# lmb-freiburg/locov

Hardware: AMD Instinct MI355X
Metric: proposals/sec through LSM ROI-head (1333x800, 1000 prop, 1203-class text bank) (higher is better)
Workload: dtype f32 (Res5 GEMM products formed from f16x2 split operands on the f16 matrix pipe, f32 accumulate; error vs f64 <= 1.5 x the f32-MFMA kernel's + 6e-7 and <= 3e-6 on every tested shape, tests/test_gpu_split_gemm.py)

## Files before the change

include/locov_hip.h:

```cpp
#ifndef LOCOV_HIP_H
#define LOCOV_HIP_H

#include <stdint.h>

#ifdef __cplusplus
extern "C" {
#endif

#define LOCOV_ABI_VERSION 8

#define LOCOV_OK 0
#define LOCOV_ERR_INVALID_ARG (-1)
#define LOCOV_ERR_LAUNCH (-2)
#define LOCOV_ERR_UNSUPPORTED (-3)

#define LOCOV_F32 0
#define LOCOV_BF16 1

#define LOCOV_NORM_NONE 0
#define LOCOV_NORM_L2 1
#define LOCOV_NORM_STANDARDIZE 2

#define LOCOV_EPI_RELU 1u
#define LOCOV_GEMM_A_SPLIT 0x1000u
// ... 428 lines not shown
} locov_weight_prep_job;
int locov_res5_weight_prep(const locov_weight_prep_job *jobs, int n_jobs, unsigned *overflow, locov_stream_t stream);

int locov_weight_transpose_scale(const float *w, int N, int K, const float *row_scale, float *out,
                                 locov_stream_t stream);
int locov_conv3x3_weight_flip(const float *w, int N, int Cin, const float *row_scale, float *out,
                              locov_stream_t stream);
int locov_im2col3x3_nhwc(const float *x, int64_t R, int H, int W, int C, float *col, locov_stream_t stream);
int locov_conv3x3_wgrad_unpack(const float *dw_packed, int N, int Cin, const float *row_scale, float *dw,
                               locov_stream_t stream);
int locov_relu_mask(const float *g, const float *act, int64_t n, float *out, float *amax_out, locov_stream_t stream);
#define LOCOV_ZERO_LIST_MAX 24
int locov_zero_if_raised(float *const *tensors, const int64_t *counts, int n_tensors, const unsigned *flag,
                         locov_stream_t stream);

int locov_spatial_mean_bwd(const float *g, const float *act, int64_t R, int C, int HW, float *out,
                           float *amax_out, locov_stream_t stream);
int locov_rows_stride2(const float *src, int N, int H, int W, int C, int forward, float *dst,
                       locov_stream_t stream);
int locov_roi_align_nhwc_bwd(const float *grad_rows, int64_t grad_ld, int N, int H, int W, int C,
                             const float *rois, int64_t R, int pooled_h, int pooled_w, float spatial_scale,
                             int sampling_ratio, int aligned, int bin_stride, int pos_major, float *grad_feat,
                             locov_stream_t stream);

#define LOCOV_REGIONS_MAX_B 64
#define LOCOV_REGIONS_MAX_CANDIDATES 4096
#define LOCOV_REGIONS_GRID 0
#define LOCOV_REGIONS_GRID_ALL 1
#define LOCOV_REGIONS_BOXES 2
#define LOCOV_REGIONS_ROWS 0
#define LOCOV_REGIONS_NCHW 1
int locov_regions_select(const double *keys, int mode, int B, const int *count_host, const int *ext_a_host,
                         const int *ext_b_host, int grid_w, const float *const *boxes_host, int n, int limit, int mask_w,
                         int mvm_w, int64_t *indices, int *src_row, int *inv, uint8_t *mask, float *loc, float *mvm,
                         locov_stream_t stream);
int locov_regions_gather_fwd(const float *src, int layout, int64_t ld, int B, int n, int C, int64_t hw, const int *src_row,
                             float *out, locov_stream_t stream);
int locov_regions_gather_bwd(const float *grad_out, int layout, int64_t ld, int64_t rows, int C, int64_t hw, const int *inv,
                             float *grad_src, locov_stream_t stream);

#define LOCOV_MHA_MAX_S 4096
#define LOCOV_MHA_MAX_GRID 65535
int locov_mha_fwd(const float *q, int64_t ldq, const float *k, int64_t ldk, const float *v, int64_t ldv, const float *bias,
                  const uint8_t *keep, float p_drop, float scale, int nseq, int S, int H, int d, float *ctx, int64_t ldo,
                  float *lse, locov_stream_t stream);
int locov_mha_bwd(const float *q, int64_t ldq, const float *k, int64_t ldk, const float *v, int64_t ldv, const float *bias,
                  const uint8_t *keep, float p_drop, float scale, int nseq, int S, int H, int d, const float *dctx,
                  int64_t ldo, const float *lse, float *delta, float *dq, int64_t lddq, float *dk, int64_t lddk, float *dv,
                  int64_t lddv, locov_stream_t stream);

int locov_resnet_stem_fwd(const float *x, int N, int H, int W, const float *w, const float *scale, const float *shift, int Cout,
                          float *y, locov_stream_t stream);

#ifdef __cplusplus
}
#endif
#endif
```

locov_amd/_lib.py:

```python
from __future__ import annotations

import ctypes
import os
from ctypes import c_char_p, c_double, c_float,c_int, c_int64, c_uint, c_void_p, POINTER

HERE = os.path.dirname(os.path.abspath(__file__))
LIB_PATH = os.environ.get("LOCOV_HIP_LIB") or os.path.join(HERE, "liblocov_hip.so")

OK = 0
F32, BF16 = 0, 1
NORM_NONE, NORM_L2, NORM_STANDARDIZE = 0, 1, 2
EPI_RELU = 1
WINO_OUT_ROI_MAJOR = 0x100
WINO_IN_ROI_MAJOR = 0x200
SEGMEAN_RES_ROI_MAJOR = 0x400
GEMM_A_SPLIT = 0x1000
EPI_OUT_SPLIT = 0x2000
EPI_RES_SPLIT = 0x4000
MAX_LEVELS = 8
ZERO_LIST_MAX = 24
LABEL_MAX_IMAGES, LABEL_MAX_THRESHOLDS, SAMPLE_MAX_PROPOSALS = 64, 6, 4096
ABI_VERSION = 8
DETECT_MAX_CANDIDATES, DETECT_FLAG_NONFINITE, DETECT_FLAG_OVERFLOW = 8192, 1, 2
RPN_FLAG_NONFINITE, RPN_MAX_PRE_NMS_TOPK, RPN_MAX_ANCHORS = 1, 16384, (1 << 22) - 1
RPN_LOSS_FLAG_DEGENERATE = 1
FED_LOSS_MAX_CLASSES = 32767
DISTILL_KD, DISTILL_JS, DISTILL_MSE, DISTILL_MAX_B = 0, 1, 2, 64
GROUNDING_ALIGN_SOFTMAX, GROUNDING_ALIGN_HARDMAX = 0, 1
TRIPLET_HARDEST, TRIPLET_EASIEST, TRIPLET_GIVEN = 0, 1, 2
BOX_IOU_GIOU, BOX_IOU_DIOU, BOX_IOU_CIOU = 0, 1, 2
REGIONS_MAX_B, REGIONS_MAX_CANDIDATES = 64, 4096
REGIONS_GRID, REGIONS_GRID_ALL, REGIONS_BOXES = 0, 1, 2
REGIONS_ROWS, REGIONS_NCHW = 0, 1
MHA_MAX_S, MHA_MAX_GRID, MHA_HEAD_DIMS = 4096, 65535, (32, 64, 96, 128)

_p = c_void_p

WEIGHT_PREP_MAX_JOBS = 32
AMAX_BOUND_MAX = 4
PREP_PLAIN, PREP_TRANSPOSE, PREP_IM2COL, PREP_IM2COL_FLIP, PREP_WINO, PREP_WINO_FLIP = range(6)


class WeightPrepJob(ctypes.Structure):
    _fields_ = [("w", c_void_p), ("row_scale", c_void_p), ("out", c_void_p), ("scale", c_float), ("kind", c_int), ("N", c_int), ("K", c_int)]


SIGNATURES = {
    "locov_abi_version": (c_int, []),
    "locov_last_error": (c_char_p, []),
    "locov_launch_count": (c_int64, []),
    "locov_device_info": (c_int, [POINTER(c_int), POINTER(c_int), POINTER(c_int)]),
    "locov_level_assign": (c_int, [_p, c_int64, c_int, c_int, c_int, c_int, _p, _p]),
    "locov_roi_align_fwd": (c_int, [_p, c_int, c_int, c_int, c_int, _p, c_int64, c_int, c_int, c_float,
                                    c_int, c_int, _p, _p]),
    "locov_roi_align_bwd": (c_int, [_p, c_int, c_int, c_int, c_int, _p, c_int64, c_int, c_int, c_float,
                                    c_int, c_int, _p, _p]),
    "locov_roi_align_levels_fwd": (c_int, [POINTER(c_void_p), POINTER(c_int), POINTER(c_int), POINTER(c_float),
                                           c_int, c_int, c_int, _p, _p, c_int64, c_int, c_int, c_int, c_int,
                                           _p, _p]),
    "locov_nchw_to_nhwc": (c_int, [_p, c_int, c_int, c_int, c_int, _p, c_int, _p]),
    "locov_roi_align_nhwc_fwd": (c_int, [_p, c_int, c_int, c_int, c_int, c_int, _p, c_int64, c_int, c_int,
                                         c_float, c_int, c_int, c_int, c_int, _p, c_int, _p]),
    "locov_roi_align_nhwc_ld_fwd": (c_int, [_p, c_int, c_int, c_int, c_int, c_int, _p, c_int64, c_int, c_int,
                                            c_float, c_int, c_int, c_int, c_int, _p, c_int64, c_int, _p]),
    "locov_roi_align_nhwc_affine_fwd": (c_int, [_p, c_int, c_int, c_int, c_int, c_int, c_int64, _p, c_int64, c_int, c_int,
                                                c_float, c_int, c_int, c_int, c_int, _p, _p, c_int, _p, c_int64, c_int, _p]),
    "locov_roi_align_from_nhwc_fwd": (c_int, [_p, c_int, c_int, c_int, c_int, _p, c_int64, c_int, c_int, c_float,
                                              c_int, c_int, _p, _p]),
    "locov_roi_align_plan_bytes": (c_int64, [c_int64]),
    "locov_roi_align_from_nhwc_fwd_ex": (c_int, [_p, c_int, c_int, c_int, c_int, _p, c_int64, c_int, c_int, c_float,
                                                 c_int, c_int, c_int, _p, c_int64, _p, _p]),
    "locov_spatial_mean_fwd": (c_int, [_p, c_int64, c_int, c_int, c_int, _p, _p]),
    "locov_gemm_nt_f32": (c_int, [_p, c_int64, _p, _p, _p, _p, _p, c_int64, c_int64, c_int, c_int, c_uint, _p]),
    "locov_conv3x3_nhwc_f32": (c_int, [_p, c_int64, c_int, c_int, c_int, c_int, _p, _p, _p, _p, _p, c_int, c_uint,
                                       _p]),
    "locov_pack_conv3x3_weight": (c_int, [_p, c_int, c_int, _p, c_int, _p]),
    "locov_winograd_workspace_bytes": (c_int64, [c_int64, c_int, c_int]),
    "locov_winograd_pack_weight": (c_int, [_p, c_int, c_int, _p, _p]),
    "locov_winograd_conv3x3_f32": (c_int, [_p, c_int64, c_int, _p, _p, _p, _p, c_int64, c_int, c_uint, _p, c_int64, _p]),
    "locov_winograd_conv3x3_f32_split": (c_int, [_p, c_int64, c_int, _p, c_float, c_float, _p, _p, _p, c_int64, c_int, c_uint,
                                                 _p, c_int64, _p, _p]),
    "locov_gemm_nt_batched_f32": (c_int, [_p, c_int64, c_int64, _p, c_int64, _p, c_int64, c_int64, c_int64, c_int,
                                          c_int, c_int, _p]),
    "locov_gemm_timing_enable": (c_int, [c_int]),
    "locov_gemm_timing_read": (c_int, [c_int, _p, _p, _p]),
    "locov_gemm_timing_read_ex": (c_int, [c_int, _p, _p, _p, _p]),
    "locov_frozen_bn_fold": (c_int, [_p, _p, _p, _p, c_float, c_int, _p, _p, _p]),
    "locov_label_proposals": (c_int, [_p, POINTER(c_int), _p, _p, POINTER(c_int), c_int, POINTER(c_float), POINTER(c_float),
                                      POINTER(c_int), c_int, c_int64, _p, _p, _p, _p, _p, _p, _p]),
    "locov_sample_proposals": (c_int, [_p, _p, _p, _p, _p, _p, _p, _p, POINTER(c_int), POINTER(c_int), c_int, c_int, c_int, c_int64,
                                       _p, _p, _p, _p, _p, _p, _p, _p]),
    "locov_box_reg_loss": (c_int, [_p, _p, _p, c_int64, _p, c_int64, c_int64, c_float, c_float, c_float, c_float, c_float, _p, _p, _p]),
    "locov_box_iou_loss": (c_int, [_p, _p, _p, c_int64, _p, c_int64, c_int64, c_float, c_float, c_float, c_float, c_double, c_int, _p, _p,
                                   _p]),
    "locov_cls_loss_workspace_bytes": (c_int64, [c_int64]),
    "locov_cls_loss": (c_int, [_p, c_int64, _p, c_int64, c_int, c_int64, _p, c_int64, _p, _p, _p, _p]),
    "locov_fed_loss_classes": (c_int, [_p, c_int64, _p, _p, c_int, c_int, _p, _p, _p]),
# ... 59 lines not shown
                                                c_int, c_int, c_float, c_float, _p, _p]),
    "locov_sim_gemm_bf16": (c_int, [_p, _p, c_int64, c_int, c_int, _p, c_int64, _p]),
    "locov_gemm_nt_f32_ex": (c_int, [_p, c_int64, _p, c_int64, _p, _p, _p, _p, _p, c_int64, c_int64, c_int, c_int, c_uint, _p]),
    "locov_conv3x3_nhwc_f32_ex": (c_int, [_p, c_int64, c_int, c_int, c_int, c_int, _p, _p, _p, _p, _p, _p, c_int, c_uint, _p]),
    "locov_winograd_conv3x3_f32_ex": (c_int, [_p, c_int64, c_int, _p, _p, _p, _p, _p, c_int64, c_int, c_uint, _p, c_int64, _p]),
    "locov_gemm_tn_workspace_bytes": (c_int64, [c_int64, c_int, c_int, c_int]),
    "locov_gemm_tn_f32": (c_int, [_p, c_int64, c_int64, _p, c_int64, c_int64, _p, c_int64, c_int64, c_int64, c_int, c_int, c_int,
                                  _p, _p, c_int64, _p]),
    "locov_split_scale_from_amax": (c_int, [_p, c_int64, c_float, _p, _p]),
    "locov_amax_bound": (c_int, [POINTER(c_void_p), POINTER(c_int64), POINTER(c_float), c_int, _p, _p]),
    "locov_split_scale_from_amax_zeroed": (c_int, [_p, c_int64, c_float, _p, _p]),
    "locov_gemm_nt_f32_split_ex": (c_int, [_p, c_int64, _p, _p, _p, _p, _p, _p, c_int64, c_int64, c_int, c_int, c_uint, c_float, _p,
                                           c_float, _p, _p, _p]),
    "locov_gemm_tn_f32_split": (c_int, [_p, c_int64, c_int64, _p, c_int64, c_int64, _p, c_int64, c_int64, c_int64, c_int, c_int, c_int,
                                        _p, _p, c_float, _p, _p, c_int64, _p]),
    "locov_gemm_tn_f32_split_b": (c_int, [_p, c_int64, c_int64, _p, c_int64, c_int64, _p, c_int64, c_int64, c_int64, c_int, c_int, c_int,
                                        _p, _p, c_float, _p, _p, c_int64, _p]),
    "locov_winograd_conv3x3_f32_split_ex": (c_int, [_p, c_int64, c_int, _p, c_float, c_float, c_int, _p, _p, _p, _p, c_int64, c_int,
                                                    c_uint, c_float, _p, c_int64, _p, _p, _p]),
    "locov_winograd_wgrad_f32_split": (c_int, [_p, _p, c_int64, c_int, c_int, c_uint, _p, _p, _p, _p, c_int64, _p]),
    "locov_winograd_wgrad_f32_split_v": (c_int, [_p, _p, c_int64, c_int, c_int, c_uint, _p, _p, _p, _p, c_int64, _p]),
    "locov_conv1x1_winograd_workspace_bytes": (c_int64, [c_int64, c_int, c_int]),
    "locov_conv1x1_winograd_workspace_bytes_for": (c_int64, [c_int64, c_int, c_int, c_int, c_int64]),
    "locov_roi_align_winograd_workspace_bytes": (c_int64, [c_int64, c_int, c_int]),
    "locov_roi_align_winograd_conv3x3_f32_split": (c_int, [_p, c_int, c_int, c_int, c_int, c_int64, _p, c_int64, c_int, c_float, c_int, c_int,
                                                           _p, _p, _p, c_float, c_float, _p, _p, _p, c_int64, c_int, c_uint, c_float, _p, c_int64,
                                                           _p, _p]),
    "locov_conv1x1_winograd_conv3x3_f32_split": (c_int, [_p, c_int64, c_int, c_float, _p, c_float, _p, _p, c_int64, c_int, _p, c_float, c_float,
                                                         _p, _p, _p, c_int64, c_int, c_uint, c_float, _p, c_int64, _p, _p]),
    "locov_winograd_wgrad_workspace_bytes": (c_int64, [c_int64, c_int, c_int]),
    "locov_winograd_wgrad_f32": (c_int, [_p, _p, c_int64, c_int, c_int, c_uint, _p, _p, _p, c_int64, _p]),
    "locov_res5_weight_prep": (c_int, [POINTER(WeightPrepJob), c_int, _p, _p]),
    "locov_weight_transpose_scale": (c_int, [_p, c_int, c_int, _p, _p, _p]),
    "locov_conv3x3_weight_flip": (c_int, [_p, c_int, c_int, _p, _p, _p]),
    "locov_im2col3x3_nhwc": (c_int, [_p, c_int64, c_int, c_int, c_int, _p, _p]),
    "locov_conv3x3_wgrad_unpack": (c_int, [_p, c_int, c_int, _p, _p, _p]),
    "locov_relu_mask": (c_int, [_p, _p, c_int64, _p, _p, _p]),
    "locov_zero_if_raised": (c_int, [POINTER(c_void_p), POINTER(c_int64), c_int, _p, _p]),
    "locov_spatial_mean_bwd": (c_int, [_p, _p, c_int64, c_int, c_int, _p, _p, _p]),
    "locov_rows_stride2": (c_int, [_p, c_int, c_int, c_int, c_int, c_int, _p, _p]),
    "locov_roi_align_nhwc_bwd": (c_int, [_p, c_int64, c_int, c_int, c_int, c_int, _p, c_int64, c_int, c_int, c_float, c_int, c_int,
                                         c_int, c_int, _p, _p]),
    "locov_box_head_fwd": (c_int, [_p, c_int64, c_int, c_int, c_int, _p, _p, _p, _p, _p, _p, c_int, c_int,
                                   c_int, c_int, _p, _p, _p, _p, _p, _p]),
    "locov_regions_select": (c_int, [_p, c_int, c_int, POINTER(c_int), POINTER(c_int), POINTER(c_int), c_int, POINTER(c_void_p), c_int, c_int,
                                     c_int, c_int, _p, _p, _p, _p, _p, _p, _p]),
    "locov_regions_gather_fwd": (c_int, [_p, c_int, c_int64, c_int, c_int, c_int, c_int64, _p, _p, _p]),
    "locov_regions_gather_bwd": (c_int, [_p, c_int, c_int64, c_int64, c_int, c_int64, _p, _p, _p]),
    "locov_mha_fwd": (c_int, [_p, c_int64, _p, c_int64, _p, c_int64, _p, _p, c_float, c_float, c_int, c_int, c_int, c_int, _p, c_int64,
                              _p, _p]),
    "locov_mha_bwd": (c_int, [_p, c_int64, _p, c_int64, _p, c_int64, _p, _p, c_float, c_float, c_int, c_int, c_int, c_int, _p,
                              c_int64, _p, _p, _p, c_int64, _p, c_int64, _p, c_int64, _p]),
    "locov_resnet_stem_fwd": (c_int, [_p, c_int, c_int, c_int, _p, _p, _p, c_int, _p, _p]),
}

_lib = None


class LocovError(RuntimeError):
    pass


def load() -> ctypes.CDLL:
    global _lib
    if _lib is not None:
        return _lib
    if not os.path.exists(LIB_PATH):
        raise LocovError(
            f"{LIB_PATH} not found: build it with `python -m locov_amd.build` "
            "(or __graft_entry__.build()).  The LSM ROI-head path has no fallback.")
    lib = ctypes.CDLL(LIB_PATH)
    for name, (restype, argtypes) in SIGNATURES.items():
        try:
            fn = getattr(lib, name)
        except AttributeError as e:
            raise LocovError(f"{LIB_PATH} does not export {name}") from e
        fn.restype = restype
        fn.argtypes = argtypes
    if lib.locov_abi_version() != ABI_VERSION:
        raise LocovError(f"ABI version mismatch: library {lib.locov_abi_version()} != binding {ABI_VERSION}")
    _lib = lib
    return lib


def check(rc: int, what: str = "") -> None:
    if rc != OK:
        msg = load().locov_last_error()
        raise LocovError(f"{what or 'liblocov_hip'} failed (code {rc}): {msg.decode() if msg else ''}")
```

locov_amd/res5.py:

```python
from __future__ import annotations

from typing import Optional

import torch
import torch.nn.functional as F
from torch import nn

import os

from .res5_operands import Res5Operands, TrainOperands

_OUT_SPLIT = os.environ.get("LOCOV_RES5_OUT_SPLIT", "1") != "0"
_FUSE12 = os.environ.get("LOCOV_RES5_FUSE12", "1") != "0"


class FrozenBatchNorm2d(nn.Module):

    def __init__(self, num_features: int, eps: float = 1e-5):
        super().__init__()
        self.num_features = num_features
        self.eps = eps
        self.register_buffer("weight", torch.ones(num_features))
        self.register_buffer("bias", torch.zeros(num_features))
        self.register_buffer("running_mean", torch.zeros(num_features))
        self.register_buffer("running_var", torch.ones(num_features) - eps)

    def scale_shift(self):
        scale = self.weight * (self.running_var + self.eps).rsqrt()
        shift = self.bias - self.running_mean * scale
        return scale, shift

    def forward(self, x):
        scale, shift = self.scale_shift()
        return x * scale.reshape(1, -1, 1, 1) + shift.reshape(1, -1, 1, 1)


class Conv2d(nn.Conv2d):

    def __init__(self, *args, norm: Optional[nn.Module] = None, **kwargs):
        super().__init__(*args, **kwargs)
        self.norm = norm

    def forward(self, x):
        x = F.conv2d(x, self.weight, self.bias, self.stride, self.padding, self.dilation, self.groups)
        if self.norm is not None:
            x = self.norm(x)
        return x


def get_norm(norm: str, ch: int):
    if norm in ("FrozenBN", "FrozenBatchNorm2d"):
        return FrozenBatchNorm2d(ch)
    if norm in ("", None):
        return None
    if norm == "BN":
        return nn.BatchNorm2d(ch)
    raise ValueError(f"unsupported norm {norm!r} for the Res5 head")


class BottleneckBlock(nn.Module):
    def __init__(self, in_channels, out_channels, *, bottleneck_channels, stride=1, num_groups=1,
                 norm="FrozenBN", stride_in_1x1=True):
        super().__init__()
        self.in_channels, self.out_channels, self.stride = in_channels, out_channels, stride
        self.stride_in_1x1 = stride_in_1x1
        if in_channels != out_channels:
            self.shortcut = Conv2d(in_channels, out_channels, kernel_size=1, stride=stride, bias=False,
                                   norm=get_norm(norm, out_channels))
        else:
            self.shortcut = None
        s1, s3 = (stride, 1) if stride_in_1x1 else (1, stride)
        self.conv1 = Conv2d(in_channels, bottleneck_channels, kernel_size=1, stride=s1, bias=False,
                            norm=get_norm(norm, bottleneck_channels))
        self.conv2 = Conv2d(bottleneck_channels, bottleneck_channels, kernel_size=3, stride=s3, padding=1,
                            bias=False, groups=num_groups, norm=get_norm(norm, bottleneck_channels))
        self.conv3 = Conv2d(bottleneck_channels, out_channels, kernel_size=1, bias=False,
                            norm=get_norm(norm, out_channels))
        for layer in (self.conv1, self.conv2, self.conv3, self.shortcut):
            if layer is not None:
                nn.init.kaiming_normal_(layer.weight, mode="fan_out", nonlinearity="relu")

    def forward(self, x):
        out = F.relu_(self.conv1(x))
        out = F.relu_(self.conv2(out))
        out = self.conv3(out)
        shortcut = self.shortcut(x) if self.shortcut is not None else x
        out = out + shortcut
        return F.relu_(out)


class Res5Stage(nn.Sequential):

    def __init__(self, *blocks):
        super().__init__(*blocks)
        self.operands = Res5Operands(self)
        self._guards = {}
        self._warned = set()

    def range_guard(self, kind: str, device):
        from . import ops
        key = (kind, torch.device(device), torch.cuda.current_stream(device).cuda_stream)
        g = self._guards.get(key)
        if g is None:
            g = self._guards[key] = ops.RangeGuard(device, deferred=kind in self.DEFERRED_KINDS)
        return g

    DEFERRED_KINDS = ("bwd", "fwd_train")

    def deferred_guards(self, device):
        dev = torch.device(device)
        return [(kind, g) for (kind, d, _), g in self._guards.items() if kind in self.DEFERRED_KINDS and d == dev]

    def backward_guard_words(self, device):
        return [g.word for kind, g in self.deferred_guards(device) if kind == "bwd"]

    def forget_scales(self) -> None:
        self.operands.forget_scales()

    def backward_guard_tripped(self) -> None:
        self.forget_scales()
        for (kind, _, _), g in self._guards.items():
            if kind == "bwd":
                g.reset()

    def backward_guard_raised(self, device) -> bool:
        words = self.backward_guard_words(device)
        hit = bool(words) and bool(int(torch.stack([w.reshape(()) for w in words]).max()))
        if hit:
            self.backward_guard_tripped()
        return hit

    def supports_rows_path(self) -> bool:
        b0 = self[0]
        return (all(isinstance(c.norm, FrozenBatchNorm2d) for blk in self for c in
                    (blk.conv1, blk.conv2, blk.conv3)) and b0.stride_in_1x1 and all(blk.conv2.groups == 1 for blk in self))

    def train_operands(self, split: bool, grid: bool = True, rois: bool = True) -> TrainOperands:
        return self.operands.train_operands(split, grid, rois)

    def rows_input(self, M: int, device) -> torch.Tensor:
        b0 = self[0]
        cin, mid = b0.conv1.in_channels, b0.conv1.out_channels
        if b0.shortcut is None or not self.supports_rows_path() or mid % 4 or cin % 4:
            return torch.empty((M, cin), dtype=torch.float32, device=device)
        buf = torch.empty((M, mid + cin), dtype=torch.float32, device=device)
        x0 = buf[:, mid:]
        x0._locov_cat = buf
        return x0

    def _linear(self, split: bool, x, conv, bias=None, tag: str = "plain", **kw):
        from . import ops
        w = self.operands.for_gemm(conv, tag, split)
        if isinstance(w, ops.SplitWeight):
            return ops.linear_split(x, w, bias, **kw)
        assert not (kw.get("x_is_split") or kw.get("out_split") or kw.get("residual_is_split")), \
            "a split-layout activation needs the split GEMM"
        for k in ("x_is_split", "x_scale", "out_split", "residual_is_split"):
            kw.pop(k, None)
        return ops.linear(x, w, bias, **kw)

    def _warn_once(self, key: str, text: str) -> None:
        if key not in self._warned:
            self._warned.add(key)
            import warnings
            warnings.warn(text, RuntimeWarning, stacklevel=3)

    ACT_SPLIT_SCALE = 16.0

    def _y2_split_ok(self, split: bool, c2, w3) -> bool:
        return bool(split) and c2.out_channels % 32 == 0 and w3.shape[1] % 32 == 0 and w3.shape[0] % 4 == 0

    def _out_split_ok(self, split: bool, winograd: bool, bi: int, pooled: bool) -> bool:
        if not (split and winograd) or bi + 1 >= len(self) or not _OUT_SPLIT:
            return False
        nxt, cur = self[bi + 1], self[bi]
        ch = cur.conv3.out_channels
        return (nxt.shortcut is None and ch % 32 == 0 and nxt.conv1.out_channels % 4 == 0 and nxt.conv3.out_channels % 8 == 0
                and nxt.conv2.in_channels % 32 == 0 and nxt.conv2.out_channels % 4 == 0)

    def map_path_pays(self, n_rois: int, n_pixels: int) -> bool:
        b0 = self[0]
        return (b0.shortcut is not None and self.supports_rows_path() and b0.conv1.in_channels % 32 == 0
                and b0.conv1.out_channels % 32 == 0 and 49 * n_rois >= 3 * n_pixels)

    @torch.no_grad()
    def forward_from_map(self, nhwc: torch.Tensor, rois: torch.Tensor, pooler_resolution: int, spatial_scale: float,
                         sampling_ratio: int = 0, aligned: bool = True, winograd: bool = True,
                         bf16: bool = False, split: bool = False, pooled: bool = False, roi_major: bool = False) -> torch.Tensor:
        from . import ops
        assert self.supports_rows_path() and self[0].shortcut is not None and pooler_resolution == 14
        b0 = self[0]
        mid = b0.conv1.out_channels
        N, H, W, cin = nhwc.shape
        P = self.operands
        wmap, shift_tail, (s1, b1) = P.get(b0, "on_map"), P.get(b0, "on_map", "shift"), P.fold(b0.conv1)
        if bf16:
            g = ops.linear_bf16(ops.to_bf16(nhwc.reshape(N * H * W, cin)), P.get(b0, "on_map", "bf16")).view(N, H, W, wmap.shape[0])
        else:
            g = self._linear(split, nhwc.reshape(N * H * W, cin), b0, tag="on_map").view(N, H, W, wmap.shape[0])
        pm = not (roi_major and not bf16)
        c2 = b0.conv2
        w3, s3, (s2, b2) = P.get(b0.conv3, "plain"), P.fold(b0.conv3)[0], P.fold(c2)
        use_wino = winograd and c2.in_channels % 32 == 0 and c2.out_channels % 4 == 0
        fuse_pool = _FUSE12 and split and use_wino and not bf16 and not pm and g.dtype == torch.float32
        R = rois.shape[0]
        y = None
        if not fuse_pool:
            y = ops.roi_align_nhwc(g[..., :mid], rois, 14, spatial_scale, sampling_ratio, aligned, bin_stride=2,
                                   pos_major=pm, ch_scale=s1, ch_shift=b1, relu=True).view(49 * R, mid)
        sc = ops.roi_align_nhwc(g[..., mid:], rois, 14, spatial_scale, sampling_ratio, aligned, bin_stride=2,
                                pos_major=pm).view(49 * R, -1)
        if bf16:
            y = ops.conv3x3_nhwc_bf16(ops.to_bf16(y), P.get(c2, "col", "bf16"), 7, 7, scale=s2, shift=b2, relu=True, pos_major=True)
            x = ops.linear_bf16(ops.to_bf16(y), P.get(b0.conv3, "plain", "bf16"), shift_tail, scale=s3, residual=sc, relu=True)
            return self.forward_rows(x, 7, 7, pos_major=True, start_block=1, bf16=True)
        y_split = False
        if use_wino:
            u2 = P.get(c2, "wino", "split" if split else "fp32")
            y_split = self._y2_split_ok(split, c2, w3)
            if fuse_pool:
                y = ops.roi_align_winograd_conv3x3(g[..., :mid], rois, 14, spatial_scale, sampling_ratio, aligned, u2,
                                                   ch_scale=s1, ch_shift=b1, scale2=s2, shift2=b2, relu=True, roi_major=True,
                                                   out_split_scale=self.ACT_SPLIT_SCALE if y_split else None)
            else:
                y = ops.winograd_conv3x3(y, u2, scale=s2, shift=b2, relu=True, roi_major=not pm, in_roi_major=not pm,
                                         out_split_scale=self.ACT_SPLIT_SCALE if y_split else None)
        else:
            y = ops.conv3x3_nhwc(y, P.get(c2, "col"), 7, 7, scale=s2, shift=b2, relu=True, pos_major=pm)
        x_split = self._out_split_ok(split, winograd, 0, pooled)
        kw3 = {"x_is_split": True, "x_scale": self.ACT_SPLIT_SCALE} if y_split else {}
        if x_split:
            kw3.update(out_split=True, x_scale=self.ACT_SPLIT_SCALE)
        x = self._linear(split, y, b0.conv3, shift_tail, scale=s3, residual=sc, relu=True, **kw3)
        return self.forward_rows(x, 7, 7, pos_major=pm, winograd=winograd, start_block=1, split=split, pooled=pooled,
                                 x0_is_split=x_split)

    @torch.no_grad()
    def forward_rows(self, x0: torch.Tensor, H: int, W: int, pos_major: bool = False,
                     winograd: bool = True, start_block: int = 0, bf16: bool = False, split: bool = False,
                     pooled: bool = False, x0_is_split: bool = False) -> torch.Tensor:
        from . import ops
        assert self.supports_rows_path(), "forward_rows needs FrozenBN, STRIDE_IN_1X1 and ungrouped convs"
        x = x0
        x_split = bool(x0_is_split)
        assert not x_split or (split and start_block > 0)
        cat = getattr(x0, "_locov_cat", None)
        P = self.operands
        for bi, blk in enumerate(self):
            if bi < start_block:
                continue
            c2 = blk.conv2
            w1, w3 = P.get(blk.conv1, "plain"), P.get(blk.conv3, "plain")
            (s1, b1), (s2, b2), (s3, b3) = P.fold(blk.conv1), P.fold(c2), P.fold(blk.conv3)
            if bf16:
                y = ops.linear_bf16(ops.to_bf16(x.contiguous()), P.get(blk.conv1, "plain", "bf16"), b1, scale=s1, relu=True)
                y = ops.conv3x3_nhwc_bf16(ops.to_bf16(y), P.get(c2, "col", "bf16"), H, W, scale=s2, shift=b2, relu=True,
                                          pos_major=pos_major)
                if blk.shortcut is not None:
                    ss, bs = P.fold(blk.shortcut)
                    sc = ops.linear_bf16(ops.to_bf16(x.contiguous()), P.get(blk.shortcut, "plain", "bf16"), bs, scale=ss)
                else:
                    sc = x
                x = ops.linear_bf16(ops.to_bf16(y), P.get(blk.conv3, "plain", "bf16"), b3, scale=s3, residual=sc, relu=True)
                continue
            xs_kw = {"x_is_split": True, "x_scale": self.ACT_SPLIT_SCALE} if x_split else {}
            use_wino = winograd and H == 7 and W == 7 and c2.in_channels % 32 == 0 and c2.out_channels % 4 == 0
            assert use_wino or not x_split
            rm = not pos_major
            fuse12 = _FUSE12 and x_split and use_wino and rm and w1.shape[0] % 32 == 0

            def conv12(**kw):
                u2 = P.get(c2, "wino", "split" if split else "fp32")
                if fuse12:
                    return ops.conv1x1_winograd_conv3x3(x, P.get(blk.conv1, "plain", "split"), b1, u2, scale1=s1, scale2=s2, shift2=b2,
                                                        relu=True, x_scale=self.ACT_SPLIT_SCALE, roi_major=kw["roi_major"],
                                                        out_split_scale=kw.get("out_split_scale"))
                return ops.winograd_conv3x3(y, u2, scale=s2, shift=b2, relu=True, in_roi_major=rm, **kw)

            y = None if fuse12 else self._linear(split, x, blk.conv1, b1, scale=s1, relu=True, **xs_kw)
            if use_wino and bi == 0 and cat is not None and blk.shortcut is not None:
                ops.winograd_conv3x3(y, P.get(c2, "wino", "split" if split else "fp32"), scale=s2, shift=b2, relu=True,
                                     out=cat[:, :c2.out_channels], roi_major=rm, in_roi_major=rm)
                x = self._linear(split, cat, blk, P.get(blk, "tail", "shift"), tag="tail", relu=True)
                continue
            last = bi == len(self) - 1
            if use_wino and pooled and last and split and blk.shortcut is None and w3.shape[1] % 32 == 0 and w3.shape[0] % 4 == 0:
                ysp = self._y2_split_ok(True, c2, w3)
                if not ops.segmean_supported(x.shape[0], w3.shape[0], w3.shape[1], H * W, residual_roi_major=rm, x_is_split=ysp,
                                             residual_is_split=x_split):
# ... 52 lines not shown
```

locov_amd/roi_heads/roi_emb_heads.py:

```python
from __future__ import annotations

import os
from typing import Dict, List, Optional

import torch
from torch import nn

from .. import ops
from ..poolers import ROIPooler, convert_boxes_to_pooler_format
from ..registry import Registry, configurable
from ..res5 import build_res5_block
from ..structures import Boxes, ShapeSpec
from .box_emb_head import build_box_predictor
from .labelling import (_EVENTS, Matcher, ROIHeads, SampleAllROIHeads, add_ground_truth_to_proposals, get_event_storage,
                        subsample_labels, subsample_order)

ROI_HEADS_REGISTRY = Registry("ROI_HEADS")
_JOINT_FORWARD = os.environ.get("LOCOV_RES5_JOINT_FWD", "1") != "0"

__all__ = ["ROI_HEADS_REGISTRY", "build_roi_heads", "Matcher", "subsample_labels", "add_ground_truth_to_proposals",
           "ROIHeads", "SampleAllROIHeads", "EmbeddingRes5ROIHeads", "EmbeddingProposalsRes5ROIHeads"]


@ROI_HEADS_REGISTRY.register()
# ... 189 lines not shown
                and self._train_path_ok(feats) and self._needs_graph(feats) and hasattr(self.res5, "range_guard")):
            return None
        if ops.active_guard(feats[0].device) is not None:
            return None
        g = self.res5.range_guard("fwd_train", feats[0].device)
        g.step_word = torch.zeros(1, dtype=torch.int32, device=feats[0].device)
        return g

    @staticmethod
    def _close_train_guard(tguard, outputs, losses=None):
        tguard.step_word.copy_(tguard.word)
        ops.zero_if_raised(list(outputs), tguard.step_word)
        return (tguard.step_word == 0).to(torch.float32).reshape(())

    def _backward_guard_tripped(self) -> None:
        import warnings
        self.res5.backward_guard_tripped()
        warnings.warn("a remembered split-operand weight scale stopped covering its weight during the previous step's Res5 backward "
                      "(weights grew 8x within 64 steps): that backward's Res5 gradients were ZEROED on the device (the step was "
                      "skipped for the Res5 weights and the feature map, GradScaler-style; no inf / NaN was applied); the scales "
                      "are chosen afresh from here on", RuntimeWarning, stacklevel=3)

    def _warn_overflow(self):
        if hasattr(self.res5, "forget_scales"):
            self.res5.forget_scales()
        if not self._overflow_warned:
            import warnings
            warnings.warn("Res5 activations left the range of the f16x2 split arithmetic (|x| >= 4094): this call was repeated "
                          "on the f32 MFMA (RES5_DTYPE 'fp32' avoids the retry; reported once per module)", RuntimeWarning, stacklevel=3)
            self._overflow_warned = True

    def _fused_roi_transform(self, features, boxes, pooled, res5_dtype):
        assert len(boxes) == features[0].shape[0]
        rois = convert_boxes_to_pooler_format(boxes)
        P = self.pooler.output_size[0]
        nhwc = ops.nchw_to_nhwc(features[0].detach())
        oh = ow = P // 2
        R = rois.shape[0]
        wino = self.res5_conv3x3 == "winograd"
        split = res5_dtype == "f16x2"
        if res5_dtype == "bf16":
            x0 = torch.empty((oh * ow * R, nhwc.shape[3]), dtype=torch.float32, device=nhwc.device)
            if P == 14 and self.res5[0].shortcut is not None:
                y = self.res5.forward_from_map(nhwc, rois, P, self.pooler.scales[0], self.pooler.sampling_ratio,
                                               self.pooler.aligned, bf16=True)
            else:
                ops.roi_align_nhwc(nhwc, rois, P, self.pooler.scales[0], self.pooler.sampling_ratio, self.pooler.aligned,
                                   bin_stride=2, pos_major=True, out=x0)
                y = self.res5.forward_rows(x0, oh, ow, pos_major=True, bf16=True)
            y = y.view(oh, ow, R, y.shape[1]).permute(2, 3, 0, 1)
            return self._pooled_mean(y) if pooled else y
        if P == 14 and self.res5.map_path_pays(R, nhwc.shape[0] * nhwc.shape[1] * nhwc.shape[2]):
            y = self.res5.forward_from_map(nhwc, rois, P, self.pooler.scales[0], self.pooler.sampling_ratio,
                                           self.pooler.aligned, winograd=wino, split=split, pooled=pooled, roi_major=wino)
            if pooled:
                return y
            return y.view(R, oh, ow, y.shape[1]).permute(0, 3, 1, 2) if wino else y.view(oh, ow, R, y.shape[1]).permute(2, 3, 0, 1)
        x0 = self.res5.rows_input(oh * ow * R, nhwc.device)
        pm = not (wino and oh == 7)
        ops.roi_align_nhwc(nhwc, rois, P, self.pooler.scales[0], self.pooler.sampling_ratio, self.pooler.aligned,
                           bin_stride=2, pos_major=pm, out=x0)
        y = self.res5.forward_rows(x0, oh, ow, pos_major=pm, winograd=wino, split=split, pooled=pooled)
        if pooled:
            return y
        return y.view(oh, ow, R, y.shape[1]).permute(2, 3, 0, 1) if pm else y.view(R, oh, ow, y.shape[1]).permute(0, 3, 1, 2)

    def _pooled_mean(self, box_features: torch.Tensor) -> torch.Tensor:
        if torch.is_grad_enabled() and box_features.requires_grad:
            return box_features.mean(dim=[2, 3])
        if not box_features.is_contiguous():
            if box_features.permute(2, 3, 0, 1).is_contiguous():
                return ops.spatial_mean(box_features.permute(2, 3, 0, 1), channels_last=2)
            if box_features.permute(0, 2, 3, 1).is_contiguous():
                return ops.spatial_mean(box_features.permute(0, 2, 3, 1), channels_last=1)
        return ops.spatial_mean(box_features)

    def forward(self, images, features, proposals, targets=None):
        del images
        if not self.training:
            del targets
            return self._detect(features, proposals)
        assert targets
        pending = self._label_begin(proposals, targets)
        del targets
        feats = [features[f] for f in self.in_features]
        del features

        def attempt(sampled):
            props = sampled if sampled is not None else self._label_finish(pending)
            proposal_boxes = [x.proposal_boxes for x in props]
            tguard = self._train_guard(feats)
            guard = None if tguard is not None else self._deferred_guard(feats)
            with ops.range_guard(tguard if tguard is not None else guard):
                box_features = self._shared_roi_transform(feats, proposal_boxes, pooled=True,
                                                          rois=pending["rois"] if pending.get("rois_of") is props else None)
            keep = None
            if tguard is not None:
                keep = self._close_train_guard(tguard, [box_features])
            elif guard is not None and guard.event is None:
                guard.snapshot()
            predictions = self.box_predictor(box_features)
            losses = self._predictor_losses(predictions, props)
            if keep is not None:
                losses = {k: v * keep for k, v in losses.items()}
            return props, losses, guard

        dtype_was = self.res5_dtype
# ... 164 lines not shown
```

Before: 393,900.

## Run the Res5 forward-from-map chain in one native call, optionally split across two streams

Adds a native res5 chain entry point that runs the on-map GEMM, ROI-align-Winograd, and the three bottleneck blocks' fused kernels from a single cached argument table. The goal is to remove Python and ctypes dispatch overhead for each stage. It can also cut the ROIs into two halves and pipeline them on a side stream offset by one stage, so kernels from the two halves overlap. INFER_SEGMENTS defaults to 1, so the default path does no split and the gain comes mainly from lower host overhead. The two-stream path adds a mutex, events, and more workspace.

```diff
diff --git a/include/locov_hip.h b/include/locov_hip.h
--- a/include/locov_hip.h
+++ b/include/locov_hip.h
@@ -504,6 +504,30 @@
 int locov_resnet_stem_fwd(const float *x, int N, int H, int W, const float *w, const float *scale, const float *shift, int Cout,
                           float *y, locov_stream_t stream);
 
+typedef struct locov_res5_chain_block {
+    const void *w1, *u2, *w3;
+    float w1_scale, u2_scale, w3_scale, pad_;
+    const float *s1, *b1, *s2, *b2, *s3, *b3;
+} locov_res5_chain_block;
+
+typedef struct locov_res5_chain {
+    const float *nhwc;
+    const float *rois;
+    const void *wmap;
+    float *g, *sc, *y, *x, *out;
+    void *wino_ws, *mean_ws;
+    unsigned *overflow;
+    int64_t R, wino_ws_bytes, mean_ws_bytes;
+    int Nimg, H, W, Cin, mid, Cout;
+    int sampling_ratio, aligned, segments, pad_;
+    float spatial_scale, wmap_scale, act_scale, v_scale;
+    locov_res5_chain_block blk[3];
+} locov_res5_chain;
+
+int locov_res5_chain_workspace_bytes(const locov_res5_chain *args_host, int64_t *wino_bytes_host, int64_t *mean_bytes_host);
+int64_t locov_res5_chain_cut(const locov_res5_chain *args_host);
+int locov_res5_chain_fwd(const locov_res5_chain *args_host, int64_t *cut_host, locov_stream_t stream);
+
 #ifdef __cplusplus
 }
 #endif
diff --git a/locov_amd/_lib.py b/locov_amd/_lib.py
--- a/locov_amd/_lib.py
+++ b/locov_amd/_lib.py
@@ -43,6 +43,23 @@
 
 class WeightPrepJob(ctypes.Structure):
     _fields_ = [("w", c_void_p), ("row_scale", c_void_p), ("out", c_void_p), ("scale", c_float), ("kind", c_int), ("N", c_int), ("K", c_int)]
+
+
+class Res5ChainBlock(ctypes.Structure):
+    _fields_ = [("w1", c_void_p), ("u2", c_void_p), ("w3", c_void_p),
+                ("w1_scale", c_float), ("u2_scale", c_float), ("w3_scale", c_float), ("pad_", c_float),
+                ("s1", c_void_p), ("b1", c_void_p), ("s2", c_void_p), ("b2", c_void_p), ("s3", c_void_p), ("b3", c_void_p)]
+
+
+class Res5Chain(ctypes.Structure):
+    _fields_ = [("nhwc", c_void_p), ("rois", c_void_p), ("wmap", c_void_p),
+                ("g", c_void_p), ("sc", c_void_p), ("y", c_void_p), ("x", c_void_p), ("out", c_void_p),
+                ("wino_ws", c_void_p), ("mean_ws", c_void_p), ("overflow", c_void_p),
+                ("R", c_int64), ("wino_ws_bytes", c_int64), ("mean_ws_bytes", c_int64),
+                ("Nimg", c_int), ("H", c_int), ("W", c_int), ("Cin", c_int), ("mid", c_int), ("Cout", c_int),
+                ("sampling_ratio", c_int), ("aligned", c_int), ("segments", c_int), ("pad_", c_int),
+                ("spatial_scale", c_float), ("wmap_scale", c_float), ("act_scale", c_float), ("v_scale", c_float),
+                ("blk", Res5ChainBlock * 3)]
 
 
 SIGNATURES = {
@@ -208,6 +225,9 @@
     "locov_mha_bwd": (c_int, [_p, c_int64, _p, c_int64, _p, c_int64, _p, _p, c_float, c_float, c_int, c_int, c_int, c_int, _p,
                               c_int64, _p, _p, _p, c_int64, _p, c_int64, _p, c_int64, _p]),
     "locov_resnet_stem_fwd": (c_int, [_p, c_int, c_int, c_int, _p, _p, _p, c_int, _p, _p]),
+    "locov_res5_chain_workspace_bytes": (c_int, [POINTER(Res5Chain), POINTER(c_int64), POINTER(c_int64)]),
+    "locov_res5_chain_cut": (c_int64, [POINTER(Res5Chain)]),
+    "locov_res5_chain_fwd": (c_int, [POINTER(Res5Chain), POINTER(c_int64), _p]),
 }
 
 _lib = None
diff --git a/locov_amd/csrc/res5_chain.hip b/locov_amd/csrc/res5_chain.hip
--- /dev/null
+++ b/locov_amd/csrc/res5_chain.hip
@@ -0,0 +1,244 @@
+#include "gemm_nt.h"
+
+#include <cstdlib>
+#include <mutex>
+
+namespace locov {
+
+namespace {
+
+constexpr int kSeg = 49;
+constexpr int kStages = 7;
+constexpr int64_t kAlign = 256;
+
+inline int64_t align_up(int64_t b) { return (b + kAlign - 1) / kAlign * kAlign; }
+
+constexpr unsigned kWinoFlags = LOCOV_EPI_RELU | LOCOV_WINO_OUT_ROI_MAJOR | LOCOV_WINO_IN_ROI_MAJOR;
+constexpr unsigned kMeanFlags = LOCOV_EPI_RELU | LOCOV_SEGMEAN_RES_ROI_MAJOR | LOCOV_GEMM_A_SPLIT | LOCOV_EPI_RES_SPLIT;
+
+struct Side {
+    std::mutex mu;
+    hipStream_t stream = nullptr;
+    hipEvent_t fork = nullptr, join = nullptr;
+};
+Side g_side[kMaxDevices];
+
+int side_of(Side **out)
+{
+    int dev = 0;
+    if (hipGetDevice(&dev) != hipSuccess || dev < 0 || dev >= kMaxDevices) return set_error(LOCOV_ERR_LAUNCH, "locov_res5_chain_fwd: hipGetDevice");
+    *out = &g_side[dev];
+    return LOCOV_OK;
+}
+
+int side_init(Side &sd)
+{
+    if (sd.stream) return LOCOV_OK;
+    hipStream_t st = nullptr;
+    hipEvent_t f = nullptr, j = nullptr;
+    if (hipStreamCreateWithFlags(&st, hipStreamNonBlocking) != hipSuccess || hipEventCreateWithFlags(&f, hipEventDisableTiming) != hipSuccess ||
+        hipEventCreateWithFlags(&j, hipEventDisableTiming) != hipSuccess) {
+        if (j) (void)hipEventDestroy(j);
+        if (f) (void)hipEventDestroy(f);
+        if (st) (void)hipStreamDestroy(st);
+        return set_error(LOCOV_ERR_LAUNCH, "locov_res5_chain_fwd: cannot create the side stream");
+    }
+    sd.stream = st, sd.fork = f, sd.join = j;
+    return LOCOV_OK;
+}
+
+unsigned tile_forms(const locov_res5_chain &a, int64_t n)
+{
+    const int64_t M = n * kSeg;
+    const Epilogue conv3{a.blk[1].s3, a.blk[1].b3, a.x, LOCOV_EPI_RELU | LOCOV_GEMM_A_SPLIT | LOCOV_EPI_OUT_SPLIT | LOCOV_EPI_RES_SPLIT};
+    const Epilogue conv1{a.blk[1].s1, a.blk[1].b1, nullptr, LOCOV_EPI_RELU | LOCOV_GEMM_A_SPLIT};
+    const Epilogue domain{nullptr, nullptr, nullptr, LOCOV_GEMM_A_SPLIT};
+    const Epilogue mean{a.blk[2].s3, a.blk[2].b3, a.sc, kMeanFlags};
+    unsigned f = 0;
+    f |= gemm_split_big_applicable(a.mid, a.Cout, M, a.Cout, a.mid, conv3, Batch{1, 0, 0, 0}, nullptr) ? 1u : 0u;
+    f |= gemm_split_big_wino_applicable(a.Cout, M, a.mid, a.Cout, conv1) ? 2u : 0u;
+    f |= gemm_split_big_applicable(a.mid, a.mid, n, a.mid, a.mid, domain, Batch{121, n * a.mid, (int64_t)a.mid * a.mid, n * a.mid}, nullptr) ? 4u : 0u;
+    f |= gemm_split_big_segmean_applicable(a.mid, M, a.Cout, a.mid, mean, kSeg) ? 8u : 0u;
+    return f;
+}
+
+int64_t choose_cut(const locov_res5_chain &a, int segments)
+{
+    if (segments < 2 || a.R < 2) return 0;
+    const unsigned whole = tile_forms(a, a.R);
+    const int64_t chunk = (whole & 8u) ? 64 : 128;
+    const int64_t cut = (a.R + chunk) / (2 * chunk) * chunk;
+    if (cut <= 0 || cut >= a.R) return 0;
+    if (tile_forms(a, cut) != whole || tile_forms(a, a.R - cut) != whole) return 0;
+    return cut;
+}
+
+int64_t wino_bytes_for(int64_t n, int mid, int Cout)
+{
+    const int64_t p = locov_roi_align_winograd_workspace_bytes(n, mid, mid), c = locov_conv1x1_winograd_workspace_bytes_for(n, Cout, mid, mid, Cout);
+    return p > c ? p : c;
+}
+
+struct Run {
+    int64_t r0, n;
+    void *wino_ws, *mean_ws;
+    int64_t wino_bytes, mean_bytes;
+    hipStream_t stream;
+};
+
+int stage(const locov_res5_chain &a, const Run &r, int k)
+{
+    const int64_t row0 = r.r0 * kSeg, M = r.n * kSeg;
+    const float *rois = a.rois + r.r0 * 5;
+    float *sc = a.sc + row0 * a.Cout, *y = a.y + row0 * a.mid, *x = a.x + row0 * a.Cout, *x1 = sc;
+    const int64_t ldg = (int64_t)a.mid + a.Cout;
+    const locov_res5_chain_block &b0 = a.blk[0], &b1 = a.blk[1], &b2 = a.blk[2];
+    locov_stream_t st = r.stream;
+    switch (k) {
+    case 0:
+        return locov_roi_align_nhwc_affine_fwd(a.g + a.mid, LOCOV_F32, a.Nimg, a.H, a.W, a.Cout, ldg, rois, r.n, 14, 14, a.spatial_scale,
+                                               a.sampling_ratio, a.aligned, 2, 0, nullptr, nullptr, 0, sc, a.Cout, LOCOV_F32, st);
+    case 1:
+        return locov_roi_align_winograd_conv3x3_f32_split(a.g, a.Nimg, a.H, a.W, a.mid, ldg, rois, r.n, 14, a.spatial_scale, a.sampling_ratio,
+                                                          a.aligned, b0.s1, b0.b1, b0.u2, b0.u2_scale, a.v_scale, b0.s2, b0.b2, y, a.mid, a.mid,
+                                                          kWinoFlags, a.act_scale, r.wino_ws, r.wino_bytes, a.overflow, st);
+    case 2:
+        return locov_gemm_nt_f32_split(y, a.mid, b0.w3, b0.s3, b0.b3, sc, x, a.Cout, M, a.Cout, a.mid,
+                                       LOCOV_EPI_RELU | LOCOV_GEMM_A_SPLIT | LOCOV_EPI_OUT_SPLIT, a.act_scale, b0.w3_scale, a.overflow, st);
+    case 3:
+        return locov_conv1x1_winograd_conv3x3_f32_split(x, a.Cout, a.Cout, a.act_scale, b1.w1, b1.w1_scale, b1.s1, b1.b1, r.n, a.mid, b1.u2,
+                                                        b1.u2_scale, a.v_scale, b1.s2, b1.b2, y, a.mid, a.mid, kWinoFlags, a.act_scale, r.wino_ws,
+                                                        r.wino_bytes, a.overflow, st);
+    case 4:
+        return locov_gemm_nt_f32_split(y, a.mid, b1.w3, b1.s3, b1.b3, x, x1, a.Cout, M, a.Cout, a.mid,
+                                       LOCOV_EPI_RELU | LOCOV_GEMM_A_SPLIT | LOCOV_EPI_OUT_SPLIT | LOCOV_EPI_RES_SPLIT, a.act_scale, b1.w3_scale,
+                                       a.overflow, st);
+    case 5:
+        return locov_conv1x1_winograd_conv3x3_f32_split(x1, a.Cout, a.Cout, a.act_scale, b2.w1, b2.w1_scale, b2.s1, b2.b1, r.n, a.mid, b2.u2,
+                                                        b2.u2_scale, a.v_scale, b2.s2, b2.b2, y, a.mid, a.mid, kWinoFlags, a.act_scale, r.wino_ws,
+                                                        r.wino_bytes, a.overflow, st);
+    default:
+        return locov_gemm_nt_f32_split_segmean(y, a.mid, b2.w3, b2.s3, b2.b3, x1, a.out + r.r0 * a.Cout, M, a.Cout, a.mid, kSeg, kMeanFlags,
+                                               a.act_scale, b2.w3_scale, r.mean_ws, r.mean_bytes, a.overflow, st);
+    }
+}
+
+int plan(const locov_res5_chain &a, int64_t cut, Run *runs, int64_t *wino_need, int64_t *mean_need)
+{
+    const int nruns = cut > 0 ? 2 : 1;
+    runs[0] = Run{0, cut > 0 ? cut : a.R, nullptr, nullptr, 0, 0, nullptr};
+    runs[1] = Run{cut, cut > 0 ? a.R - cut : 0, nullptr, nullptr, 0, 0, nullptr};
+    int64_t wino_off = 0, mean_off = 0;
+    *wino_need = *mean_need = 0;
+    for (int i = 0; i < nruns; i++) {
+        Run &r = runs[i];
+        r.wino_bytes = wino_bytes_for(r.n, a.mid, a.Cout);
+        r.mean_bytes = locov_gemm_segmean_workspace_bytes(r.n * kSeg, a.Cout);
+        r.wino_ws = static_cast<char *>(a.wino_ws) + wino_off;
+        r.mean_ws = static_cast<char *>(a.mean_ws) + mean_off;
+        *wino_need = wino_off + r.wino_bytes;
+        *mean_need = mean_off + r.mean_bytes;
+        wino_off += align_up(r.wino_bytes);
+        mean_off += align_up(r.mean_bytes);
+    }
+    return nruns;
+}
+
+int requested_segments(int segments)
+{
+    const char *e = getenv("LOCOV_INFER_SEGMENTS");
+    return e && *e ? atoi(e) : segments;
+}
+
+}
+
+}
+
+using namespace locov;
+
+extern "C" {
+
+int locov_res5_chain_workspace_bytes(const locov_res5_chain *args_host, int64_t *wino_bytes_host, int64_t *mean_bytes_host)
+{
+    LOCOV_REQUIRE(args_host && wino_bytes_host && mean_bytes_host, "locov_res5_chain_workspace_bytes: null pointer");
+    const locov_res5_chain &a = *args_host;
+    const int segments = requested_segments(a.segments);
+    LOCOV_REQUIRE(segments == 1 || segments == 2, "locov_res5_chain_workspace_bytes: segments must be 1 or 2 (got %d)", segments);
+    LOCOV_REQUIRE(a.R >= 0 && a.mid > 0 && a.Cout > 0, "locov_res5_chain_workspace_bytes: bad shape");
+    Run one[2], two[2];
+    int64_t w1 = 0, m1 = 0, w2 = 0, m2 = 0;
+    plan(a, 0, one, &w1, &m1);
+    plan(a, choose_cut(a, segments), two, &w2, &m2);
+    *wino_bytes_host = w1 > w2 ? w1 : w2;
+    *mean_bytes_host = m1 > m2 ? m1 : m2;
+    return LOCOV_OK;
+}
+
+int64_t locov_res5_chain_cut(const locov_res5_chain *args_host)
+{
+    LOCOV_REQUIRE(args_host, "locov_res5_chain_cut: null argument table");
+    const int segments = requested_segments(args_host->segments);
+    LOCOV_REQUIRE(segments == 1 || segments == 2, "locov_res5_chain_cut: segments must be 1 or 2 (got %d)", segments);
+    LOCOV_REQUIRE(args_host->R >= 0 && args_host->mid > 0 && args_host->Cout > 0, "locov_res5_chain_cut: bad shape");
+    return choose_cut(*args_host, segments);
+}
+
+int locov_res5_chain_fwd(const locov_res5_chain *args_host, int64_t *cut_host, locov_stream_t stream)
+{
+    LOCOV_REQUIRE(args_host, "locov_res5_chain_fwd: null argument table");
+    const locov_res5_chain &a = *args_host;
+    const int segments = requested_segments(a.segments);
+    LOCOV_REQUIRE(segments == 1 || segments == 2, "locov_res5_chain_fwd: segments must be 1 or 2 (got %d)", segments);
+    LOCOV_REQUIRE(a.R >= 0 && a.Nimg > 0 && a.H > 0 && a.W > 0 && a.Cin > 0 && a.mid > 0 && a.Cout > 0, "locov_res5_chain_fwd: bad shape");
+    if (cut_host) *cut_host = 0;
+    if (a.R == 0) return LOCOV_OK;
+    LOCOV_REQUIRE(a.nhwc && a.rois && a.wmap && a.g && a.sc && a.y && a.x && a.out && a.wino_ws && a.mean_ws, "locov_res5_chain_fwd: null pointer");
+    LOCOV_REQUIRE(a.Cin % 32 == 0 && a.mid % 32 == 0 && a.Cout % 32 == 0, "locov_res5_chain_fwd: Cin, mid and Cout must be multiples of 32");
+    LOCOV_REQUIRE(a.act_scale > 0.f && a.v_scale > 0.f && a.wmap_scale > 0.f && a.spatial_scale > 0.f, "locov_res5_chain_fwd: scales must be positive");
+    for (int b = 0; b < 3; b++)
+        LOCOV_REQUIRE((b == 0 || a.blk[b].w1) && a.blk[b].u2 && a.blk[b].w3, "locov_res5_chain_fwd: null operand in block %d", b);
+
+    hipStream_t main_stream = as_stream(stream);
+    int64_t cut = choose_cut(a, segments);
+    if (cut > 0) {
+        hipStreamCaptureStatus cs = hipStreamCaptureStatusNone;
+        if (hipStreamIsCapturing(main_stream, &cs) != hipSuccess || cs != hipStreamCaptureStatusNone) cut = 0;
+    }
+    Run runs[2];
+    int64_t wino_need = 0, mean_need = 0;
+    const int nruns = plan(a, cut, runs, &wino_need, &mean_need);
+    runs[0].stream = main_stream;
+    for (int i = 0; i < nruns; i++)
+        if (!locov_gemm_segmean_supported(a.mid, runs[i].n * kSeg, a.Cout, a.mid, kSeg, kMeanFlags))
+            return set_error(LOCOV_ERR_UNSUPPORTED, "locov_res5_chain_fwd: the mean-fused convolution cannot take %lld rows x %d channels",
+                             (long long)(runs[i].n * kSeg), a.Cout);
+    LOCOV_REQUIRE(wino_need <= a.wino_ws_bytes && mean_need <= a.mean_ws_bytes, "locov_res5_chain_fwd: workspace too small (%lld / %lld bytes)",
+                  (long long)a.wino_ws_bytes, (long long)a.mean_ws_bytes);
+    LOCOV_REQUIRE(((uintptr_t)a.wino_ws | (uintptr_t)a.mean_ws) % 16 == 0, "locov_res5_chain_fwd: misaligned workspace");
+
+    int rc = locov_gemm_nt_f32_split(a.nhwc, a.Cin, a.wmap, nullptr, nullptr, nullptr, a.g, (int64_t)a.mid + a.Cout, (int64_t)a.Nimg * a.H * a.W,
+                                     a.mid + a.Cout, a.Cin, 0u, a.act_scale, a.wmap_scale, a.overflow, stream);
+    if (rc) return rc;
+    if (nruns == 1) {
+        for (int k = 0; k < kStages && !rc; k++) rc = stage(a, runs[0], k);
+        return rc;
+    }
+
+    Side *sd = nullptr;
+    if ((rc = side_of(&sd))) return rc;
+    std::lock_guard<std::mutex> lock(sd->mu);
+    if ((rc = side_init(*sd))) return rc;
+    runs[1].stream = sd->stream;
+    if (hipEventRecord(sd->fork, main_stream) != hipSuccess || hipStreamWaitEvent(sd->stream, sd->fork, 0) != hipSuccess)
+        return set_error(LOCOV_ERR_LAUNCH, "locov_res5_chain_fwd: fork failed");
+    for (int t = 0; t <= kStages && !rc; t++) {
+        if (t < kStages) rc = stage(a, runs[0], t);
+        if (!rc && t >= 1) rc = stage(a, runs[1], t - 1);
+    }
+    if (hipEventRecord(sd->join, sd->stream) != hipSuccess || hipStreamWaitEvent(main_stream, sd->join, 0) != hipSuccess)
+        return rc ? rc : set_error(LOCOV_ERR_LAUNCH, "locov_res5_chain_fwd: join failed");
+    if (!rc && cut_host) *cut_host = cut;
+    return rc;
+}
+
+}
diff --git a/locov_amd/res5.py b/locov_amd/res5.py
--- a/locov_amd/res5.py
+++ b/locov_amd/res5.py
@@ -8,10 +8,12 @@
 
 import os
 
-from .res5_operands import Res5Operands, TrainOperands
+from .res5_operands import Res5Operands, TrainOperands, conv_version
 
 _OUT_SPLIT = os.environ.get("LOCOV_RES5_OUT_SPLIT", "1") != "0"
 _FUSE12 = os.environ.get("LOCOV_RES5_FUSE12", "1") != "0"
+_CHAIN = os.environ.get("LOCOV_RES5_CHAIN", "1") != "0"
+INFER_SEGMENTS = 1
 
 
 class FrozenBatchNorm2d(nn.Module):
@@ -96,6 +98,8 @@
         self.operands = Res5Operands(self)
         self._guards = {}
         self._warned = set()
+        self.last_cut = 0
+        self._chain = None
 
     def range_guard(self, kind: str, device):
         from . import ops
@@ -186,9 +190,12 @@
     @torch.no_grad()
     def forward_from_map(self, nhwc: torch.Tensor, rois: torch.Tensor, pooler_resolution: int, spatial_scale: float,
                          sampling_ratio: int = 0, aligned: bool = True, winograd: bool = True,
-                         bf16: bool = False, split: bool = False, pooled: bool = False, roi_major: bool = False) -> torch.Tensor:
+                         bf16: bool = False, split: bool = False, pooled: bool = False, roi_major: bool = False,
+                         segments: Optional[int] = None) -> torch.Tensor:
         from . import ops
         assert self.supports_rows_path() and self[0].shortcut is not None and pooler_resolution == 14
+        if _CHAIN and pooled and roi_major and not bf16 and self._chain_ok(nhwc, rois, split, winograd):
+            return self._forward_chain(nhwc, rois, spatial_scale, sampling_ratio, aligned, INFER_SEGMENTS if segments is None else segments)
         b0 = self[0]
         mid = b0.conv1.out_channels
         N, H, W, cin = nhwc.shape
@@ -235,6 +242,93 @@
         return self.forward_rows(x, 7, 7, pos_major=pm, winograd=winograd, start_block=1, split=split, pooled=pooled,
                                  x0_is_split=x_split)
 
+    def _chain_ok(self, nhwc: torch.Tensor, rois: torch.Tensor, split: bool, winograd: bool) -> bool:
+        from . import ops
+        if not (split and winograd and _FUSE12 and _OUT_SPLIT and len(self) == 3 and rois.shape[0] > 0 and nhwc.is_cuda
+                and nhwc.dtype == torch.float32 and nhwc.is_contiguous() and rois.dtype == torch.float32 and rois.is_cuda):
+            return False
+        b0, b1, b2 = self
+        cin, mid, cout = b0.conv1.in_channels, b0.conv1.out_channels, b0.conv3.out_channels
+        if b1.shortcut is not None or b2.shortcut is not None or cin % 32 or mid % 32 or cout % 32:
+            return False
+        for bi, blk in enumerate(self):
+            if (blk.conv1.in_channels, blk.conv1.out_channels, blk.conv2.in_channels, blk.conv2.out_channels, blk.conv3.in_channels,
+                    blk.conv3.out_channels) != (cout if bi else cin, mid, mid, mid, mid, cout):
+                return False
+        if not (self._out_split_ok(True, True, 0, True) and self._out_split_ok(True, True, 1, True)):
+            return False
+        return ops.segmean_supported(49 * rois.shape[0], cout, mid, 49, residual_roi_major=True, x_is_split=True, residual_is_split=True)
+
+    def _chain_table(self):
+        from . import _lib
+        P = self.operands
+        b0 = self[0]
+        mark = P.entries.get((b0, "on_map"))
+        versions = tuple(conv_version(c) for blk in self for c in (blk.conv1, blk.conv2, blk.conv3, blk.shortcut) if c is not None)
+        hit = self._chain
+        if hit is not None and hit[0] == versions and hit[1] is mark and mark is not None and "split" in mark:
+            return hit[2]
+        keep = []
+
+        def ptr(t):
+            keep.append(t)
+            return t.data_ptr()
+
+        tab = _lib.Res5Chain()
+        wmap = P.for_gemm(b0, "on_map", True)
+        shift_tail = P.get(b0, "on_map", "shift")
+        tab.wmap, tab.wmap_scale = ptr(wmap.data), wmap.scale
+        tab.Cin, tab.mid, tab.Cout = b0.conv1.in_channels, b0.conv1.out_channels, b0.conv3.out_channels
+        tab.act_scale, tab.v_scale = self.ACT_SPLIT_SCALE, 0.25
+        for bi, blk in enumerate(self):
+            e = tab.blk[bi]
+            (s1, b1), (s2, b2), (s3, b3) = P.fold(blk.conv1), P.fold(blk.conv2), P.fold(blk.conv3)
+            u2 = P.get(blk.conv2, "wino", "split")
+            if bi:
+                w1 = P.get(blk.conv1, "plain", "split")
+                e.w1, e.w1_scale = ptr(w1.data), w1.scale
+            w3 = P.for_gemm(blk.conv3, "plain", True) if bi < 2 else P.get(blk.conv3, "plain", "split")
+            e.u2, e.u2_scale, e.w3, e.w3_scale = ptr(u2.data), u2.scale, ptr(w3.data), w3.scale
+            e.s1, e.b1, e.s2, e.b2, e.s3 = ptr(s1), ptr(b1), ptr(s2), ptr(b2), ptr(s3)
+            e.b3 = ptr(shift_tail if bi == 0 else b3)
+        for t in keep:
+            assert t.is_contiguous() and t.dtype == torch.float32 and t.data_ptr() % 16 == 0
+        self._chain = (versions, P.entries.get((b0, "on_map")), tab, keep)
+        return tab
+
+    def _forward_chain(self, nhwc: torch.Tensor, rois: torch.Tensor, spatial_scale: float, sampling_ratio: int, aligned: bool,
+                       segments: int = 1) -> torch.Tensor:
+        import ctypes
+        from . import _lib, ops
+        lib = _lib.load()
+        base = self._chain_table()
+        tab = _lib.Res5Chain()
+        ctypes.memmove(ctypes.byref(tab), ctypes.byref(base), ctypes.sizeof(tab))
+        N, H, W, cin = nhwc.shape
+        assert cin == tab.Cin
+        rois = rois.contiguous()
+        R, dev = rois.shape[0], nhwc.device
+        tab.Nimg, tab.H, tab.W, tab.R, tab.segments = N, H, W, R, int(segments)
+        tab.spatial_scale, tab.sampling_ratio, tab.aligned = float(spatial_scale), int(sampling_ratio), int(aligned)
+        wino_b, mean_b = ctypes.c_int64(), ctypes.c_int64()
+        _lib.check(lib.locov_res5_chain_workspace_bytes(ctypes.byref(tab), ctypes.byref(wino_b), ctypes.byref(mean_b)),
+                   "locov_res5_chain_workspace_bytes")
+        f32 = dict(dtype=torch.float32, device=dev)
+        g = torch.empty((N * H * W, tab.mid + tab.Cout), **f32)
+        sc, x = torch.empty((49 * R, tab.Cout), **f32), torch.empty((49 * R, tab.Cout), **f32)
+        y, out = torch.empty((49 * R, tab.mid), **f32), torch.empty((R, tab.Cout), **f32)
+        wino_ws = torch.empty(max(wino_b.value, 16), dtype=torch.uint8, device=dev)
+        mean_ws = torch.empty(max(mean_b.value, 16), dtype=torch.uint8, device=dev)
+        word = ops._overflow_word(nhwc)
+        tab.nhwc, tab.rois, tab.overflow = nhwc.data_ptr(), rois.data_ptr(), word.data_ptr()
+        tab.g, tab.sc, tab.x, tab.y, tab.out = g.data_ptr(), sc.data_ptr(), x.data_ptr(), y.data_ptr(), out.data_ptr()
+        tab.wino_ws, tab.wino_ws_bytes, tab.mean_ws, tab.mean_ws_bytes = wino_ws.data_ptr(), wino_ws.numel(), mean_ws.data_ptr(), mean_ws.numel()
+        cut = ctypes.c_int64()
+        with torch.cuda.device(dev):
+            _lib.check(lib.locov_res5_chain_fwd(ctypes.byref(tab), ctypes.byref(cut), ops._stream(nhwc)), "locov_res5_chain_fwd")
+        self.last_cut = cut.value
+        return out
+
     @torch.no_grad()
     def forward_rows(self, x0: torch.Tensor, H: int, W: int, pos_major: bool = False,
                      winograd: bool = True, start_block: int = 0, bf16: bool = False, split: bool = False,
diff --git a/locov_amd/roi_heads/roi_emb_heads.py b/locov_amd/roi_heads/roi_emb_heads.py
--- a/locov_amd/roi_heads/roi_emb_heads.py
+++ b/locov_amd/roi_heads/roi_emb_heads.py
@@ -265,7 +265,8 @@
             return self._pooled_mean(y) if pooled else y
         if P == 14 and self.res5.map_path_pays(R, nhwc.shape[0] * nhwc.shape[1] * nhwc.shape[2]):
             y = self.res5.forward_from_map(nhwc, rois, P, self.pooler.scales[0], self.pooler.sampling_ratio,
-                                           self.pooler.aligned, winograd=wino, split=split, pooled=pooled, roi_major=wino)
+                                           self.pooler.aligned, winograd=wino, split=split, pooled=pooled, roi_major=wino,
+                                           segments=1 if len(boxes) == 1 else None)
             if pooled:
                 return y
             return y.view(R, oh, ow, y.shape[1]).permute(0, 3, 1, 2) if wino else y.view(oh, ow, R, y.shape[1]).permute(2, 3, 0, 1)
```

After: 396,800, median of 6. About the same (+0.7%).
